# AutomationLabs-sh/AutomationLabsModelPredictiveControl.jl

Hardware: AMD Instinct MI355X
Metric: MPC steps/s (batch=4096, nx=12, nu=4, N=30) (higher is better)
Workload: dtype f64; 1 GPU; configs[1]: hover-linearised quadrotor nx=12 nu=4 N=30, 4096 instances per GPU, shared model, x0 amplitude classes 0.3/1.0/3.0 interleaved, cold start every step; batch_per_gpu=4096, global_batch=4096, seed=0x5eed0002, setup_ramp_steps=300, admm_max_iter=6, check_every=6, polish=1, warm_state_kept=False, parallelism=instances sharded over 1 GPU(s), 16-instance tile per workgroup

## Files before the change

automationlabsmodelpredictivecontrol.jl_amd/csrc/almpc_kernels.hip.h:

```cpp
#pragma once
#include <hip/hip_runtime.h>
#include <stdint.h>

#include <map>
#include <mutex>
#include <utility>
#include <type_traits>

namespace almpc {

inline hipError_t ensure_dyn_lds(const void* fn, size_t bytes) {
    if (bytes <= 64 * 1024) return hipSuccess;
    static std::mutex mu;
    static std::map<std::pair<int, const void*>, size_t> cur;
    int dev = 0;
    hipError_t e = hipGetDevice(&dev);
    if (e != hipSuccess) return e;
    std::lock_guard<std::mutex> lock(mu);
    size_t& c = cur[std::make_pair(dev, fn)];
    if (c >= bytes) return hipSuccess;
    e = hipFuncSetAttribute(fn, hipFuncAttributeMaxDynamicSharedMemorySize, (int)bytes);
    if (e == hipSuccess) c = bytes;
    return e;
}
// ... 587 lines not shown
    const double f = piv ? -invd : col * invd;
    const double keep = piv ? 0.0 : 1.0;
#pragma unroll
    for (int jj = 0; jj < 16; ++jj) r[jj] = __builtin_fma(-f, pj[jj], keep * r[jj]);
    if (own) r[JJ] = f;
}

template <int JJ>
__device__ __forceinline__ void gj16_pivot2(gj16_row& r, const double (&pj0)[16], const double (&pj1)[16], const double col0, const double col1,
                                            const double i11, const double t, const double s22, const bool own, const int k, const int lane) {
    static_assert((JJ & 1) == 0 && JJ + 1 < 16, "a pair starts at an even position");
    const double e11 = fast_rcp_d(s22);
    const double e01 = -t * e11;
    const double e00 = __builtin_fma(-t, e01, i11);
    const bool p0 = lane == k, p1 = lane == k + 1;
    double f0 = __builtin_fma(col0, e00, col1 * e01), f1 = __builtin_fma(col0, e01, col1 * e11);
    f0 = p0 ? -e00 : (p1 ? -e01 : f0);
    f1 = p0 ? -e01 : (p1 ? -e11 : f1);
    const double keep = (p0 || p1) ? 0.0 : 1.0;
#pragma unroll
    for (int jj = 0; jj < 16; ++jj) r[jj] = __builtin_fma(-f1, pj1[jj], __builtin_fma(-f0, pj0[jj], keep * r[jj]));
    if (own) { r[JJ] = f0; r[JJ + 1] = f1; }
}

template <int I, int N, class F>
__device__ __forceinline__ void gj_static_for(F&& f) {
    if constexpr (I < N) {
        if (!f(std::integral_constant<int, I>{})) return;
        gj_static_for<I + 1, N>(f);
    }
}

__device__ __forceinline__ void wave_lds_sync() {
    __builtin_amdgcn_fence(__ATOMIC_RELEASE, "workgroup");
    __builtin_amdgcn_wave_barrier();
    __builtin_amdgcn_fence(__ATOMIC_ACQUIRE, "workgroup");
}

template <int CTRL, int ROW_MASK>
__device__ __forceinline__ double dpp_d(double v) {
    int lo = __double2loint(v), hi = __double2hiint(v);
    lo = __builtin_amdgcn_update_dpp(lo, lo, CTRL, ROW_MASK, 0xF, false);
    hi = __builtin_amdgcn_update_dpp(hi, hi, CTRL, ROW_MASK, 0xF, false);
    return __hiloint2double(hi, lo);
}
#define ALMPC_WAVE_REDUCE(NAME, OP)                                                     \
    __device__ __forceinline__ double NAME(double v) {                                  \
        v = OP(v, dpp_d<0x121, 0xF>(v));                                 \
        v = OP(v, dpp_d<0x122, 0xF>(v));                                 \
        v = OP(v, dpp_d<0x124, 0xF>(v));                                 \
        v = OP(v, dpp_d<0x128, 0xF>(v));                                 \
        { const double o = dpp_d<0x142, 0xA>(v);           \
          const bool take = ((threadIdx.x >> 4) & 1) != 0; v = take ? OP(v, o) : v; }   \
        { const double o = dpp_d<0x143, 0xC>(v);           \
          const bool take = ((threadIdx.x >> 5) & 1) != 0; v = take ? OP(v, o) : v; }   \
        return readlane_d(v, 63);                                                       \
    }
__device__ __forceinline__ double op_add(double a, double b) { return a + b; }
__device__ __forceinline__ double op_min(double a, double b) { return fmin(a, b); }
__device__ __forceinline__ double op_max(double a, double b) { return fmax(a, b); }
ALMPC_WAVE_REDUCE(wave_sum, op_add)
ALMPC_WAVE_REDUCE(wave_min, op_min)
ALMPC_WAVE_REDUCE(wave_max, op_max)
#undef ALMPC_WAVE_REDUCE

__device__ __forceinline__ double half_sum(double v) {
    const unsigned lo = (unsigned)__double2loint(v), hi = (unsigned)__double2hiint(v);
    const auto a = __builtin_amdgcn_permlane32_swap(lo, lo, false, false);
    const auto b = __builtin_amdgcn_permlane32_swap(hi, hi, false, false);
    return __hiloint2double((int)b[0], (int)a[0]) + __hiloint2double((int)b[1], (int)a[1]);
}

__device__ __forceinline__ void lds_barrier() {
    __builtin_amdgcn_fence(__ATOMIC_RELEASE, "workgroup", "local");
    __builtin_amdgcn_s_barrier();
    __builtin_amdgcn_fence(__ATOMIC_ACQUIRE, "workgroup", "local");
}

template <class T>
__device__ __forceinline__ T* GL(T* q) {
    return (T*)(__attribute__((address_space(1))) T*)q;
}

__device__ __forceinline__ void wave_fence_lds() {
    __builtin_amdgcn_fence(__ATOMIC_RELEASE, "wavefront");
    __builtin_amdgcn_wave_barrier();
    __builtin_amdgcn_fence(__ATOMIC_ACQUIRE, "wavefront");
}

struct RowMultOut {
    double* mu = nullptr;
    const int* done = nullptr;
    const double* mer = nullptr;
};
__device__ __forceinline__ bool row_mult_live(const RowMultOut& r, int inst) {
    return r.mu != nullptr && !(r.done && r.done[inst] != 0) && !(r.mer && r.mer[4 * (size_t)inst + 2] != 0.0);
}

template <bool GLB>
struct PolishMode {
    static constexpr bool glb = GLB;
    static constexpr bool half = !GLB;
    static constexpr int WL = GLB ? 64 : 32;
    static constexpr int PMASK = WL - 1;
};

template <int CPL>
__device__ __forceinline__ void rollout_steps(double* Z, int n, int m, int N, int G, int lane, const double* A,
                                              const double* B) {
    const int C = n + m;
    const int i = lane / G, g = lane % G;
    double coef[CPL];
    int jc[CPL];
#pragma unroll
    for (int t = 0; t < CPL; ++t) {
        const int j = g * CPL + t;
        const bool ok = (i < n) && (j < C);
        const int ic = i < n ? i : 0;
        const double av = A[(size_t)(j < n ? j : 0) * n + ic], bv = B[(size_t)((j >= n && j < C) ? j - n : 0) * n + ic];
        coef[t] = ok ? (j < n ? av : bv) : 0.0;
        jc[t] = j < C ? j : C - 1;
    }
    for (int k = 0; k < N; ++k) {
        const double* zk = Z + (size_t)k * C;
        double zv[CPL];
#pragma unroll
        for (int t = 0; t < CPL; ++t) zv[t] = zk[jc[t]];
        double acc = 0.0;
#pragma unroll
        for (int t = 0; t < CPL; ++t) acc += coef[t] * zv[t];
        if (G == 4) {
            acc += dpp_d<0xB1, 0xF>(acc);
            acc += dpp_d<0x4E, 0xF>(acc);
        } else {
            for (int o = 1; o < G; o <<= 1) acc += __shfl_xor(acc, o);
        }
        if (g == 0 && i < n) Z[(size_t)(k + 1) * C + i] = acc;
        __builtin_amdgcn_fence(__ATOMIC_RELEASE, "wavefront");
        __builtin_amdgcn_wave_barrier();
        __builtin_amdgcn_fence(__ATOMIC_ACQUIRE, "wavefront");
    }
}

constexpr int ROLL_SMX = 24, ROLL_NX = 16;
template <int SMX, int NX>
__device__ __forceinline__ void roll_load(const double* M, int lane, double (&cu)[SMX], double (&cx)[NX]) {
#pragma unroll
    for (int c = 0; c < SMX; ++c) cu[c] = M[c * 64 + lane];
#pragma unroll
    for (int c = 0; c < NX; ++c) cx[c] = M[(ROLL_SMX + c) * 64 + lane];
}
template <int SMX, int NX>
__device__ __forceinline__ void roll_run(const double (&cu)[SMX], const double (&cx)[NX], int n, int m, int N, int s, int nb, int lane,
                                         const double* eub, double e0v, double x0r, const double* xref_lds, const double* xref_glb,
                                         double* gx, double* gex) {
    const int nx = n * (N + 1), sm = s * m;
    if (lane < n) {
        gex[lane] = e0v;
        if (gx) gx[lane] = x0r;
    }
    const bool mine = lane < s * n;
    auto upart = [&](int b, double (&acc)[4]) {
        const double* ub = eub + b * sm;
        double uv[SMX];
#pragma unroll
        for (int c = 0; c < SMX; ++c) uv[c] = ub[c];
#pragma unroll
        for (int t = 0; t < 4; ++t) acc[t] = 0.0;
#pragma unroll
        for (int c = 0; c < SMX; ++c) acc[c & 3] = __builtin_fma(cu[c], uv[c], acc[c & 3]);
    };
    double acc[4];
    upart(0, acc);
    double prev = e0v;
    int src0 = 0;
#pragma unroll 1
    for (int b = 0; b < nb; ++b) {
        const int t = (b * s + 1) * n + lane;
        const bool ok = mine && t < nx;
        const int tc = ok ? t : 0;
        double xr;
        if (xref_lds) xr = xref_lds[tc];
        else xr = xref_glb[tc];
#pragma unroll
        for (int c = 0; c < NX; ++c) {
            const int sl = src0 + c;
            acc[c & 3] = __builtin_fma(cx[c], readlane_d(prev, sl < 64 ? sl : 63), acc[c & 3]);
        }
        const double ev = (acc[0] + acc[1]) + (acc[2] + acc[3]);
        prev = ev;
        src0 = (s - 1) * n;
        upart(b + 1, acc);
        if (xref_lds) asm volatile("" : "+v"(xr));
        if (ok) {
            gex[t] = ev;
            if (gx) gx[t] = ev + xr;
        }
    }
}

constexpr int POLISH_WAVES = 4;
#ifndef ALMPC_EXP_POLISH_WAVES
#define ALMPC_EXP_POLISH_WAVES 8
#endif
constexpr int POLISH_WAVES_GLDS = ALMPC_EXP_POLISH_WAVES;
constexpr int POLISH_LDS_MIN_PER_WAVE = 128 + 64 + 64 + 32;
struct PolishShared {
    int off_d, off_umin, off_umax, off_uref, off_ab, off_xref, total;
};
__host__ __device__ inline PolishShared polish_shared_layout(int n, int m, int N, int nz, int nzs, int fused) {
    PolishShared L;
    L.off_d = 0;
    L.off_umin = nzs;
    L.off_umax = L.off_umin + m;
    L.off_uref = L.off_umax + m;
    L.off_ab = L.off_uref + nz;
    L.off_xref = L.off_ab + ((fused && fused != 3) ? n * (n + m) : 0);
    L.total = (L.off_xref + (fused ? (N + 1) * n : 0) + 1) & ~1;
    return L;
}
constexpr int POLISH_GLB_PER_INST = 64 * 64;
constexpr int POLISH_SG_SHARED_CAP = 48;
constexpr int HANDOFF_REC = POLISH_LDS_MIN_PER_WAVE;
static_assert((TILE - 8) * HANDOFF_REC <= POLISH_SG_SHARED_CAP * 64, "the records of ranks 8..15 must fit the second-tier slot");

typedef double d2 __attribute__((ext_vector_type(2)));

template <bool GLDS, bool GPRE, int KOFF, bool SGL = false, bool START = false>
__device__ __forceinline__ void polish_body(const PolishParams& p_arg, double* smem) {
    const PolishParams& p = p_arg;
    constexpr int CH = (GLDS || SGL) ? 8 : 16;
    constexpr int NWV = GLDS ? POLISH_WAVES_GLDS : (SGL ? 1 : POLISH_WAVES);
    const int wv = __builtin_amdgcn_readfirstlane(threadIdx.x >> 6), lane_k = threadIdx.x & 63;
    const int nz = p.nz, nzs = p.nzs;
    const double* Gp = p.G;
    const int gs = GLDS ? ((nz + 1) & ~1) : nzs;
    const PolishShared SL = polish_shared_layout(p.roll.n, p.m, p.roll.N, nz, nzs, p.fuse_rollout);
    double* shc = smem + (GLDS ? (size_t)nz * gs : 0);
    double* wave_lds = shc + SL.total + (size_t)wv * p.lds_per_wave;
    int* qcnt = nullptr;
    const bool uref_sh = p.uref_stride == 0, xref_sh = p.roll.xref_stride == 0;
    const bool per_inst = p.G_stride != 0;
    double* cd = shc + SL.off_d;
    double* cab = shc + SL.off_ab;
    if (per_inst) { cd = wave_lds + p.wave_const_off; cab = cd + nzs; }
    bool handed = false;
    if constexpr (GLDS && GPRE) handed = p.handoff != 0;
    if (!handed) {
        constexpr int TPB = 64 * NWV;
        const int n = p.roll.n, m = p.m, N = p.roll.N;
        if (!per_inst)
            for (int t = threadIdx.x; t < nzs; t += TPB) shc[SL.off_d + t] = p.dvec[t];
        for (int t = threadIdx.x; t < m; t += TPB) { shc[SL.off_umin + t] = p.umin[t]; shc[SL.off_umax + t] = p.umax[t]; }
        if (uref_sh)
            for (int t = threadIdx.x; t < nz; t += TPB) shc[SL.off_uref + t] = p.uref[t];
        if (p.fuse_rollout) {
            if (!per_inst && p.fuse_rollout != 3) {
                for (int t = threadIdx.x; t < n * n; t += TPB) shc[SL.off_ab + t] = p.roll.A[t];
                for (int t = threadIdx.x; t < n * m; t += TPB) shc[SL.off_ab + n * n + t] = p.roll.B[t];
            }
            if (xref_sh)
                for (int t = threadIdx.x; t < (N + 1) * n; t += TPB) shc[SL.off_xref + t] = p.roll.xref[t];
        }
    }
    ALMPC_STAMP(8192 + blockIdx.x * 8 + wv, 0);
    if constexpr (GLDS && !GPRE) {
        const int hs = gs / 2;
        const bool lane_in = lane_k < hs;
        const int lq = lane_in ? lane_k : 0;
        for (int r0_ = wv; r0_ < nz; r0_ += POLISH_WAVES_GLDS * 8) {
            d2 v[8];
#pragma unroll
            for (int u = 0; u < 8; ++u) {
                const int r = r0_ + u * POLISH_WAVES_GLDS;
                v[u] = *reinterpret_cast<const d2*>(p.G + (size_t)(r < nz ? r : 0) * nzs + 2 * lq);
            }
#pragma unroll
            for (int u = 0; u < 8; ++u) {
                const int r = r0_ + u * POLISH_WAVES_GLDS;
                if (r < nz && lane_in) *reinterpret_cast<d2*>(smem + (size_t)r * gs + 2 * lq) = v[u];
            }
        }
    }
    if constexpr (GLDS) {
        qcnt = reinterpret_cast<int*>(shc + SL.total + (size_t)POLISH_WAVES_GLDS * p.lds_per_wave);
        if (!handed && threadIdx.x == 0) { qcnt[0] = POLISH_WAVES_GLDS; qcnt[1] = -1; qcnt[2] = 0; }
        Gp = smem;
    }
    if (!handed) __syncthreads();
#ifdef ALMPC_EXP_LANE_GEOMETRY_PER_INSTANCE
    constexpr bool GEO_ONCE = false;
#else
    constexpr bool GEO_ONCE = CH == 8;
#endif
    [[maybe_unused]] int geo_m0 = 0;
    if constexpr (GEO_ONCE) geo_m0 = (2 * lane_k) % p.m;
  auto process = [&](const int inst, const double* rec, const int rank) {
    auto ka_ = __builtin_amdgcn_kernarg_segment_ptr();
    asm volatile("" : "+s"(ka_));
    const PolishParams& p = *(const PolishParams*)((const char*)ka_ + KOFF);
    int lane = lane_k;
    asm volatile("" : "+v"(lane));
    ALMPC_STAMP(inst, 8);
    if constexpr (!GLDS) {
        if (per_inst) {
            if constexpr (SGL) {
                double* gl = wave_lds + p.g_off;
                const char* src = reinterpret_cast<const char*>(GL(p.G) + (size_t)inst * p.G_stride) + lane * 16;
                if (lane < nzs / 2)
                    for (int r = 0; r < nz; ++r)
                        __builtin_amdgcn_global_load_lds((const __attribute__((address_space(1))) void*)(src + (size_t)r * nzs * 8),
                                                         (__attribute__((address_space(3))) void*)(gl + (size_t)r * nzs), 16, 0, 0);
                Gp = gl;
            } else
            Gp = GL(p.G) + (size_t)inst * p.G_stride;
            const int n_ = p.roll.n, m_ = p.m;
            for (int t = lane; t < nzs; t += 64) cd[t] = GL(p.dvec)[(size_t)inst * p.d_stride + t];
            if (p.fuse_rollout) {
                for (int t = lane; t < n_ * n_; t += 64) cab[t] = GL(p.roll.A)[(size_t)inst * p.A_stride + t];
                for (int t = lane; t < n_ * m_; t += 64) cab[n_ * n_ + t] = GL(p.roll.B)[(size_t)inst * p.B_stride + t];
            }
            if constexpr (SGL) __builtin_amdgcn_s_waitcnt(0);
            wave_fence_lds();
        }
    }
    bool from_rec = false;
    if constexpr (GLDS && GPRE) from_rec = rec != nullptr;
    int st_in;
    if (from_rec) st_in = __builtin_amdgcn_readfirstlane(reinterpret_cast<const int*>(rec + 256)[HANDOFF_STATUS]);
    else st_in = GL(p.status)[inst];
    const size_t base = (size_t)inst * nzs;
    const int r0 = 2 * lane, r1 = 2 * lane + 1;
    const bool in0 = r0 < nz, in1 = r1 < nz;
    const bool inrow = r0 < nzs;
    const int rc = inrow ? r0 : 0;
    const bool skip = (st_in == 2);
    int im0;
    if constexpr (GEO_ONCE) im0 = geo_m0; else im0 = r0 % p.m;
    const int im1 = (im0 + 1 == p.m) ? 0 : im0 + 1;

    double* rowbuf = wave_lds;
    double* pbufa = rowbuf + 128;
    double* pbufb = pbufa + 64;
    int* wrow_s = reinterpret_cast<int*>(pbufb + 64);
#ifdef ALMPC_EXP_ROW_NUMBERS
    auto woff = [&](int row) { return row; };
    auto wadr = [&](int e) { return e * gs; };
#else
    auto woff = [&](int row) { return row * gs; };
    auto wadr = [&](int e) { return e; };
#endif
    double* Sg;
    int cap2 = 64;
    bool own_slot = false;
    const bool sg_lds = SGL && p.sg_off >= 0;
    if (sg_lds) Sg = wave_lds + p.sg_off;
    else Sg = GL(p.sglobal) + (size_t)inst * POLISH_GLB_PER_INST;

    double lo0 = 0, hi0 = 0, lo1 = 0, hi1 = 0, v00, v01, w0 = 0, w1 = 0, y0, y1, z0, z1;
    double x0r = 0.0;
    if (p.fuse_rollout && lane < p.roll.n) x0r = GL(p.roll.x0)[(size_t)inst * p.roll.n + lane];
    {
        const d2 dv = *reinterpret_cast<const d2*>(cd + rc);
        d2 vv, yy, zz;
        if (from_rec) {
            const int o = (rc + handoff_rot(rank)) & 127;
            zz = *reinterpret_cast<const d2*>(rec + o);
            vv = *reinterpret_cast<const d2*>(rec + 128 + o);
            uint32_t wd = (uint32_t)reinterpret_cast<const int*>(rec + 256)[rc >> 4];
            asm volatile("" : "+v"(zz), "+v"(vv), "+v"(wd));
            const uint32_t b = (uint32_t)(rc & 15);
            yy[0] = (double)(int)((wd >> (16u + b)) & 1u) - (double)(int)((wd >> b) & 1u);
            yy[1] = (double)(int)((wd >> (17u + b)) & 1u) - (double)(int)((wd >> (b + 1u)) & 1u);
            if (rank >= POLISH_WAVES_GLDS) {
                __builtin_amdgcn_fence(__ATOMIC_RELEASE, "workgroup");
                if (lane == 0) atomicSub(qcnt + 2, 1);
// ... 508 lines not shown
                        pbufa[hpos] = Sr[tj];
                        pbufb[hpos] = (hpos < pv) ? -Sr[tj] : Sr[tj];
                    }
                    wave_fence_lds();
                    const double fcol = pbufa[hpos], piv = pbufa[pv];
                    double rowpv[16];
                    bcast16(pbufb, rowpv);
                    const double ip = fast_rcp_d(piv);
                    const bool isp = hpos == pv;
                    const double f = isp ? 0.0 : fcol * ip;
                    const double scale = isp ? ip : 1.0;
#pragma unroll
                    for (int t = 0; t < 16; ++t) Sr[t] = __builtin_fma(-f, rowpv[t], Sr[t]) * scale;
                    Sr[tj] = (hhf == hh) ? (isp ? ip : -f) : Sr[tj];
                }
            }
        }
        recompute(m);
        if (pass == 1 || k0 > 32) break;
        {
            const bool mine = lane < 32 && pos < k;
            const double viol = mine ? ((wsd > 0) ? -lam : lam) : -__builtin_inf();
            const double lmax = wave_max(mine ? fabs(lam) : 0.0);
            const bool bad = mine && viol > 1e-12 * fmax(1.0, lmax);
            const unsigned badm = (unsigned)__ballot(bad);
            const int nb = __popc(badm);
            if (nb < 2) break;
            const unsigned usedm = (k >= 32) ? 0xffffffffu : ((1u << k) - 1u);
            const unsigned keepm = usedm & ~badm;
            put_rows(0.0, 0.0);
            if (bad) rowbuf[wrow] = 1.0;
            wave_fence_lds();
            {
                const d2 mk = *reinterpret_cast<const d2*>(rowbuf + r0);
                if (mk[0] != 0.0) act0 = false;
                if (mk[1] != 0.0) act1 = false;
            }
            const bool keep = lane < 32 && ((keepm >> pos) & 1u) != 0u;
            const int np = __popc(keepm & ((1u << pos) - 1u));
            if (keep) { ibuf[np] = wrow; ibuf[64 + np] = wsd; pbufa[np] = wbnd; }
            wave_fence_lds();
            k = __popc(keepm);
            wrow = 0; wsd = 0; wbnd = 0.0; lam = 0.0;
            if (pos < k) { wrow = ibuf[pos]; wsd = ibuf[64 + pos]; wbnd = pbufa[pos]; }
            wave_fence_lds();
            it += nb;
        }
        }
        if (k0 > 32) {
            tier2_home(k0);
            to_global();
            for (int q = 32; q < k0; ++q)
                add_row(PolishMode<true>{}, __builtin_amdgcn_readlane(pend_row, q), readlane_d(pend_bnd, q),
                        __builtin_amdgcn_readlane(pend_sd, q));
            fresh = false;
            overflow = true;
        }
        }
    }
    ALMPC_STAMP(inst, 10);
    if (!give_up) {
        if (!overflow) {
            run(PolishMode<false>{});
            if (overflow) { tier2_home(33); to_global(); }
        }
        if (overflow) {
            overflow = false;
            run(PolishMode<true>{});
            if (overflow && own_slot) {
                slot_to_global();
                overflow = false;
                run(PolishMode<true>{});
            }
            give_up = overflow;
        }
    }
    if constexpr (GLDS) {
        if (own_slot) {
            if (lane == 0) atomicExch(qcnt + 1, -1);
            own_slot = false;
        }
    }

    ALMPC_STAMP(inst, 11);
    ALMPC_ACC_FLUSH(inst);
    d2 wout;
    if (p.unsolved && lane == 0 && ((give_up || fin != 0) ? st_in : 0) != 0) {
        __hip_atomic_fetch_add(p.unsolved, 1, __ATOMIC_RELAXED, __HIP_MEMORY_SCOPE_SYSTEM);
        if (p.redo_gate) *GL(p.redo_gate) = p.step_serial;
    }
    if (give_up) {
        wout[0] = skip ? z0 : fmin(fmax(z0, lo0), hi0);
        wout[1] = skip ? z1 : fmin(fmax(z1, lo1), hi1);
    } else {
        wout[0] = act0 ? bnd0 : fmin(fmax(w0, lo0), hi0);
        wout[1] = act1 ? bnd1 : fmin(fmax(w1, lo1), hi1);
        if (lane == 0) {
            GL(p.piters)[inst] = it;
            GL(p.status)[inst] = (fin == 0) ? 0 : st_in;
        }
    }
    if (p.dflag && lane == 0 && GL(p.dflag)[inst] != 0) GL(p.status)[inst] = 2;
    if (!p.fuse_rollout) {
        if (inrow) *reinterpret_cast<d2*>(GL(p.w) + base + r0) = wout;
        return;
    }
    {
        const RolloutParams& rp = p.roll;
        const int n = rp.n, m = rp.m, N = rp.N, C = n + m;
        double* Z = wave_lds;
        const d2 dvp = *reinterpret_cast<const d2*>(cd + rc);
        double ur0 = 0.0, ur1 = 0.0;
        if (uref_sh) {
            ur0 = shc[SL.off_uref + (in0 ? r0 : 0)];
            ur1 = shc[SL.off_uref + (in1 ? r1 : 0)];
            asm volatile("" : "+v"(ur0), "+v"(ur1));
        } else {
            const double* ug = GL(rp.uref) + (size_t)inst * rp.uref_stride;
            ur0 = ug[in0 ? r0 : 0];
            ur1 = ug[in1 ? r1 : 0];
        }
        if (p.fuse_rollout == 3) {
            const bool exact = p.roll_s * m <= 20 && n <= 12;
            double cu[ROLL_SMX], cx[ROLL_NX];
            if (exact) {
                double cu2[20], cx2[12];
                roll_load<20, 12>(GL(p.rollM), lane, cu2, cx2);
#pragma unroll
                for (int c = 0; c < ROLL_SMX; ++c) cu[c] = c < 20 ? cu2[c] : 0.0;
#pragma unroll
                for (int c = 0; c < ROLL_NX; ++c) cx[c] = c < 12 ? cx2[c] : 0.0;
            } else {
                roll_load<ROLL_SMX, ROLL_NX>(GL(p.rollM), lane, cu, cx);
            }
            const int m0 = im0, m1 = im1;
            double e0 = 0.0, e1 = 0.0;
            if (in0) {
                const double uu = fmin(fmax(wout[0] * dvp[0] + ur0, shc[SL.off_umin + m0]), shc[SL.off_umax + m0]);
                e0 = uu - ur0;
                GL(rp.u)[(size_t)inst * nz + r0] = uu;
                GL(rp.eu)[(size_t)inst * nz + r0] = e0;
            }
            if (in1) {
                const double uu = fmin(fmax(wout[1] * dvp[1] + ur1, shc[SL.off_umin + m1]), shc[SL.off_umax + m1]);
                e1 = uu - ur1;
                GL(rp.u)[(size_t)inst * nz + r1] = uu;
                GL(rp.eu)[(size_t)inst * nz + r1] = e1;
            }
            double* eub = wave_lds;
            {
                d2 ev; ev[0] = e0; ev[1] = e1;
                *reinterpret_cast<d2*>(eub + 2 * lane) = ev;
                d2 zz; zz[0] = 0.0; zz[1] = 0.0;
                *reinterpret_cast<d2*>(eub + 128 + 2 * lane) = zz;
            }
            double e0v = 0.0;
            const double* xg = nullptr;
            if (lane < n) {
                double xr0;
                if (xref_sh) { xr0 = shc[SL.off_xref + lane]; asm volatile("" : "+v"(xr0)); }
                else xr0 = GL(rp.xref)[(size_t)inst * rp.xref_stride + lane];
                e0v = x0r - xr0;
            }
            if (!xref_sh) xg = GL(rp.xref) + (size_t)inst * rp.xref_stride;
            wave_fence_lds();
            ALMPC_STAMP(inst, 12);
            const size_t xo3 = (size_t)inst * n * (N + 1);
            double* gx = GL(rp.x) + xo3;
            double* gex = GL(rp.ex) + xo3;
            const double* xl = xref_sh ? (shc + SL.off_xref) : nullptr;
            if (exact) {
                double cu2[20], cx2[12];
#pragma unroll
                for (int c = 0; c < 20; ++c) cu2[c] = cu[c];
#pragma unroll
                for (int c = 0; c < 12; ++c) cx2[c] = cx[c];
                roll_run<20, 12>(cu2, cx2, n, m, N, p.roll_s, p.roll_nb, lane, eub, e0v, x0r, xl, xg, gx, gex);
            } else {
                roll_run<ROLL_SMX, ROLL_NX>(cu, cx, n, m, N, p.roll_s, p.roll_nb, lane, eub, e0v, x0r, xl, xg, gx, gex);
            }
            ALMPC_STAMP(inst, 13);
            ALMPC_STAMP(inst, 14);
            return;
        }
        const int m0 = im0, m1 = im1, k0s = r0 / m, k1s = (m0 + 1 == m) ? k0s + 1 : k0s;
        if (in0) {
            const double uu = fmin(fmax(wout[0] * dvp[0] + ur0, shc[SL.off_umin + m0]), shc[SL.off_umax + m0]);
            GL(rp.u)[(size_t)inst * nz + r0] = uu;
            GL(rp.eu)[(size_t)inst * nz + r0] = uu - ur0;
            Z[(size_t)k0s * C + n + m0] = uu - ur0;
        }
        if (in1) {
            const double uu = fmin(fmax(wout[1] * dvp[1] + ur1, shc[SL.off_umin + m1]), shc[SL.off_umax + m1]);
            GL(rp.u)[(size_t)inst * nz + r1] = uu;
            GL(rp.eu)[(size_t)inst * nz + r1] = uu - ur1;
            Z[(size_t)k1s * C + n + m1] = uu - ur1;
        }
        if (p.fuse_rollout == 2) return;
        if (lane < n) {
            double xr0;
            if (xref_sh) { xr0 = shc[SL.off_xref + lane]; asm volatile("" : "+v"(xr0)); }
            else xr0 = GL(rp.xref)[(size_t)inst * rp.xref_stride + lane];
            Z[lane] = x0r - xr0;
        }
        wave_fence_lds();
        ALMPC_STAMP(inst, 12);
        switch (p.roll_cpl) {
            case 1: rollout_steps<1>(Z, n, m, N, p.roll_g, lane, cab, cab + n * n); break;
            case 2: rollout_steps<2>(Z, n, m, N, p.roll_g, lane, cab, cab + n * n); break;
            case 4: rollout_steps<4>(Z, n, m, N, p.roll_g, lane, cab, cab + n * n); break;
            default: rollout_steps<8>(Z, n, m, N, p.roll_g, lane, cab, cab + n * n); break;
        }
        ALMPC_STAMP(inst, 13);
        const int nx = n * (N + 1);
        const size_t xo = (size_t)inst * nx;
        const float inv_n = 1.0f / (float)n;
        for (int t0 = 0; t0 < nx; t0 += 4 * 64) {
            double ev[4], xr[4];
            int tt[4];
#pragma unroll
            for (int u = 0; u < 4; ++u) {
                const int t = t0 + 64 * u + lane;
                tt[u] = t < nx ? t : nx - 1;
                const int kq = (int)(((float)tt[u] + 0.5f) * inv_n);
                ev[u] = Z[(size_t)tt[u] + (size_t)kq * m];
            }
            if (xref_sh) {
#pragma unroll
                for (int u = 0; u < 4; ++u) xr[u] = shc[SL.off_xref + tt[u]];
                asm volatile("" : "+v"(xr[0]), "+v"(xr[1]), "+v"(xr[2]), "+v"(xr[3]));
            } else {
                const double* xg = GL(rp.xref) + (size_t)inst * rp.xref_stride;
#pragma unroll
                for (int u = 0; u < 4; ++u) xr[u] = xg[tt[u]];
            }
#pragma unroll
            for (int u = 0; u < 4; ++u) {
                const int t = t0 + 64 * u + lane;
                if (t < nx) {
                    GL(rp.ex)[xo + t] = ev[u];
                    GL(rp.x)[xo + t] = (t < n) ? x0r : ev[u] + xr[u];
                }
            }
        }
        ALMPC_STAMP(inst, 14);
    }
  };

    if constexpr (GLDS) {
        ALMPC_STAMP(8192 + blockIdx.x * 8 + wv, 1);
        [[maybe_unused]] int nproc = 0;
        for (int i = wv;;) {
            const int tile = (i >> 4) * (int)gridDim.x + (int)blockIdx.x;
            if (tile >= p.ntiles) break;
            int inst;
            const double* rec = nullptr;
            if (handed) {
                if (i >= p.batch - (int)blockIdx.x * TILE) break;
                rec = i < POLISH_WAVES_GLDS ? wave_lds : shc + p.sg_shared_off + (size_t)(i - POLISH_WAVES_GLDS) * HANDOFF_REC;
                inst = __builtin_amdgcn_readfirstlane(reinterpret_cast<const int*>(rec + 256)[HANDOFF_INST]);
            } else {
                inst = p.perm[tile * 16 + (i & 15)];
            }
            if (inst >= 0) {
                process(inst, rec, i);
                ++nproc;
// ... 185 lines not shown
```

automationlabsmodelpredictivecontrol.jl_amd/csrc/almpc_polish_gen.hip.h:

```cpp
#pragma once
#include "almpc_kernels.hip.h"

namespace almpc {

struct PolishGenParams {
    int nz, mc, R, Rs, m, n, N, batch, nzs;
    const double* Ghat;
    const double* gnorm;
    long Ghat_stride = 0, gnorm_stride = 0, d_stride = 0, A_stride = 0, B_stride = 0;
    int ltv = 0;
    const double* ltvA = nullptr;
    const double* ltvB = nullptr;
    const double* ltvC = nullptr;
    const double* eq_off = nullptr;
    long eq_stride = 0;
    const double* rollM = nullptr;
    int roll_s = 0, roll_nb = 0;
    int eq_proj = 0, eq0 = 0, ne = 0;
    const double* GhatE = nullptr;
    const double* WinvE = nullptr;
    const int* row_traj;
    const int* row_eq;
    const int* row_xidx;
    const int* row_state;
// ... 742 lines not shown
    if (lane == 0) {
        p.piters[inst] = it;
        const int st_out = (st_in == 2) ? 2 : ((fin == 0) ? 0 : (fin == 3 ? 3 : 1));
        p.status[inst] = st_out;
        const bool requeue = !QUEUE && overflow && fin != 3;
        if (requeue) p.ovf[2 + atomicAdd(p.ovf, 1)] = inst;
        if (p.unsolved && st_out == 1 && !requeue) {
            __hip_atomic_fetch_add(p.unsolved, 1, __ATOMIC_RELAXED, __HIP_MEMORY_SCOPE_SYSTEM);
            if (p.redo_gate) *p.redo_gate = p.step_serial;
        }
    }
    if (p.redo_ws) {
        const int st_out = (st_in == 2) ? 2 : ((fin == 0) ? 0 : (fin == 3 ? 3 : 1));
        const bool requeue = !QUEUE && overflow && fin != 3;
        int32_t* rw = p.redo_ws + (size_t)inst * 64;
        if (st_out == 1 && !requeue && k > 0) {
            const int pos = WL == 32 ? (lane & 31) : lane;
            if (lane < WL && pos < k && pos < 63) {
                const int xi = p.row_xidx[wrow];
                const int t = wrow < p.nz ? (wrow / p.m) * p.redo_sp + p.redo_nt + wrow % p.m : (xi / p.n) * p.redo_sp + xi % p.n;
                rw[1 + pos] = (t << 2) | (wsd == 0 ? 2 : (wsd > 0 ? 1 : 0));
            }
            if (lane == 0) rw[0] = k < 63 ? k : 63;
        } else if (lane == 0) rw[0] = 0;
    }
    if (!QUEUE && overflow && fin != 3) {
        if (lane < 32) p.ovf_ws[(size_t)inst * 32 + lane] = guess_overflow ? -1 : (wrow | ((wsd + 1) << 12));
        if (p.ovf_sinv && !guess_overflow) {
            double* sv_ = p.ovf_sinv + (size_t)inst * (32 * 32 + 32);
#pragma unroll 4
            for (int t = 0; t < 32; t += 2) sv_[(t + (lane >> 5)) * 32 + (lane & 31)] = Sl[(t + (lane >> 5)) * WL + (lane & 31)];
            if (lane < 32) sv_[32 * 32 + lane] = wbnd;
        }
    }
    wave_fence_lds();
    if (p.rows.mu && fin == 0 && st_in != 2 && row_mult_live(p.rows, inst)) {
#pragma unroll
        for (int q = 0; q < NP; ++q) {
            d2 v; v[0] = 0.0; v[1] = 0.0;
            *reinterpret_cast<d2*>(rowbuf + 2 * lane + 128 * q) = v;
        }
        wave_fence_lds();
        if (lowhalf && pos < k && wrow >= nz) rowbuf[wrow] = lam;
        wave_fence_lds();
        double* mo = p.rows.mu + (size_t)inst * N * n;
        for (int t = lane; t < N * n; t += 64) {
            const int r = p.rows_map[t];
            mo[t] = r >= 0 ? rowbuf[nz + r] : 0.0;
        }
        wave_fence_lds();
    }
    {
        const int r0 = 2 * lane, r1 = 2 * lane + 1;
        const int rc = (r0 < nzs) ? r0 : 0;
        const d2 dvp = *reinterpret_cast<const d2*>(dvi + rc);
        if (r0 < nz) {
            const double ur = rp.uref[(size_t)inst * rp.uref_stride + r0];
            const double uu = fmin(fmax(wout[0] * dvp[0] + ur, rp.umin[r0 % m]), rp.umax[r0 % m]);
            rp.u[(size_t)inst * nz + r0] = uu;
            rp.eu[(size_t)inst * nz + r0] = uu - ur;
            Z[(size_t)(r0 / m) * C + n + r0 % m] = uu - ur;
        }
        if (r1 < nz) {
            const double ur = rp.uref[(size_t)inst * rp.uref_stride + r1];
            const double uu = fmin(fmax(wout[1] * dvp[1] + ur, rp.umin[r1 % m]), rp.umax[r1 % m]);
            rp.u[(size_t)inst * nz + r1] = uu;
            rp.eu[(size_t)inst * nz + r1] = uu - ur;
            Z[(size_t)(r1 / m) * C + n + r1 % m] = uu - ur;
        }
        if (blocked) {
            {
                d2 ev;
                ev[0] = (r0 < nz) ? Z[(size_t)(r0 / m) * C + n + r0 % m] : 0.0;
                ev[1] = (r1 < nz) ? Z[(size_t)(r1 / m) * C + n + r1 % m] : 0.0;
                wave_fence_lds();
                *reinterpret_cast<d2*>(EUB + 2 * lane) = ev;
                d2 zz; zz[0] = 0.0; zz[1] = 0.0;
                *reinterpret_cast<d2*>(EUB + 128 + 2 * lane) = zz;
            }
            double e0v = 0.0, x0r = 0.0;
            if (lane < n) { x0r = rp.x0[(size_t)inst * n + lane]; e0v = x0r - rp.xref[(size_t)inst * rp.xref_stride + lane]; }
            double cu[ROLL_SMX], cx[ROLL_NX];
            roll_load<ROLL_SMX, ROLL_NX>(p.rollM, lane, cu, cx);
            wave_fence_lds();
            PGEN_STAMP(13);
            const size_t xo = (size_t)inst * n * (N + 1);
            roll_run<ROLL_SMX, ROLL_NX>(cu, cx, n, m, N, p.roll_s, p.roll_nb, lane, EUB, e0v, x0r, nullptr,
                                        rp.xref + (size_t)inst * rp.xref_stride, rp.x + xo, rp.ex + xo);
            PGEN_STAMP(14);
        } else if (!p.ltv) {
        for (int i = lane; i < n; i += 64) Z[i] = rp.x0[(size_t)inst * n + i] - rp.xref[(size_t)inst * rp.xref_stride + i];
        wave_fence_lds();
        PGEN_STAMP(13);
        roll(Z);
        PGEN_STAMP(14);
        const int nx = n * (N + 1);
        const size_t xo = (size_t)inst * nx;
        for (int t0 = 0; t0 < nx; t0 += 256) {
            double xr4[4];
#pragma unroll
            for (int j = 0; j < 4; ++j) {
                const int t = t0 + 64 * j + lane, tc = t < nx ? t : 0;
                xr4[j] = (tc < n) ? rp.x0[(size_t)inst * n + tc] : rp.xref[(size_t)inst * rp.xref_stride + tc];
            }
#pragma unroll
            for (int j = 0; j < 4; ++j) {
                const int t = t0 + 64 * j + lane;
                if (t < nx) {
                    const double ev = Z[(size_t)(t / n) * C + t % n];
                    rp.ex[xo + t] = ev;
                    rp.x[xo + t] = (t < n) ? xr4[j] : ev + xr4[j];
                }
            }
        }
        }
    }
    PGEN_STAMP(6);
    if (QUEUE) wave_fence_lds();
  } while (QUEUE);
}

struct GhatInstParams {
    int n, m, N, nz, nzs, mc, R, Rs;
    const double* A; const double* B;
    long A_stride, B_stride;
    long A_kstride, B_kstride;
    const double* G; long G_stride;
    const double* dvec; long d_stride;
    const int* rowmap;
    double* Ghat; long Ghat_stride;
    double* gnorm; long gnorm_stride;
};
constexpr int GHAT_THREADS = 256;

template <int NX>
__global__ __launch_bounds__(GHAT_THREADS) void k_ghat_inst(GhatInstParams p) {
    extern __shared__ __attribute__((aligned(16))) double smem[];
    const int inst = blockIdx.x, tid = threadIdx.x;
    const int n = p.n, m = p.m, N = p.N, nz = p.nz, nzs = p.nzs, mc = p.mc, R = p.R, Rs = p.Rs;
    double* AB = smem;
    const double* G = p.G + (size_t)inst * p.G_stride;
    const double* dv = p.dvec + (size_t)inst * p.d_stride;
    double* Gh = p.Ghat + (size_t)inst * p.Ghat_stride;
    double* gn = p.gnorm + (size_t)inst * p.gnorm_stride;
    for (int t = tid; t < nz * nz; t += GHAT_THREADS) Gh[(size_t)(t / nz) * Rs + t % nz] = G[(size_t)(t / nz) * nzs + t % nz];
    for (int pass = 0; pass < 2; ++pass) {
        const int ncol = pass == 0 ? nz : mc;
        for (int c0 = 0; c0 < ncol; c0 += GHAT_THREADS) {
            const int c = c0 + tid;
            const bool on = c < ncol;
            const int cc = on ? c : 0;
            double x[NX];
#pragma unroll
            for (int i = 0; i < NX; ++i) x[i] = 0.0;
            for (int t = 0; t < N; ++t) {
                if (t == 0 || p.A_kstride != 0) {
                    __syncthreads();
                    const double* At = p.A + (size_t)inst * p.A_stride + (size_t)t * p.A_kstride;
                    const double* Bt = p.B + (size_t)inst * p.B_stride + (size_t)t * p.B_kstride;
                    for (int e = tid; e < n * n; e += GHAT_THREADS) AB[e] = At[e];
                    for (int e = tid; e < n * m; e += GHAT_THREADS) AB[n * n + e] = Bt[e];
                    __syncthreads();
                }
                double xn[NX];
#pragma unroll
                for (int i = 0; i < NX; ++i) xn[i] = 0.0;
#pragma unroll
                for (int j = 0; j < NX; ++j)
                    if (j < n) {
                        const double xj = x[j];
#pragma unroll
// ... 126 lines not shown
```

Baseline: 18700 batch-steps/s (one step = 4096 instance QP solves).

## Restructure fused polish rollout tail to overlap loads and prefetch xref

Moves the fuse_rollout==3 tail ahead of the status writes. It issues the rollout matrix loads early, hoists the kernel arguments into scalar registers once, and places a waitcnt before the tail so those loads overlap with the u/eu stores and status writes. roll_run now prefetches the next block's xref value one iteration ahead. It uses explicit global and LDS address-space pointers, with template tags replacing the runtime LDS/global branch. The exact-size register arrays are loaded directly instead of through copies into padded arrays. The risk is higher register pressure and subtle ordering issues around the waitcnt and the asm barriers.

```diff
diff --git a/automationlabsmodelpredictivecontrol.jl_amd/csrc/almpc_kernels.hip.h b/automationlabsmodelpredictivecontrol.jl_amd/csrc/almpc_kernels.hip.h
--- a/automationlabsmodelpredictivecontrol.jl_amd/csrc/almpc_kernels.hip.h
+++ b/automationlabsmodelpredictivecontrol.jl_amd/csrc/almpc_kernels.hip.h
@@ -693,6 +693,11 @@
     return (T*)(__attribute__((address_space(1))) T*)q;
 }
 
+template <class T>
+__device__ __forceinline__ __attribute__((address_space(1))) T* G1(T* q) {
+    return (__attribute__((address_space(1))) T*)q;
+}
+
 __device__ __forceinline__ void wave_fence_lds() {
     __builtin_amdgcn_fence(__ATOMIC_RELEASE, "wavefront");
     __builtin_amdgcn_wave_barrier();
@@ -757,20 +762,30 @@
 template <int SMX, int NX>
 __device__ __forceinline__ void roll_load(const double* M, int lane, double (&cu)[SMX], double (&cx)[NX]) {
 #pragma unroll
-    for (int c = 0; c < SMX; ++c) cu[c] = M[c * 64 + lane];
-#pragma unroll
-    for (int c = 0; c < NX; ++c) cx[c] = M[(ROLL_SMX + c) * 64 + lane];
-}
-template <int SMX, int NX>
+    for (int c = 0; c < SMX; ++c) cu[c] = G1(M)[c * 64 + lane];
+#pragma unroll
+    for (int c = 0; c < NX; ++c) cx[c] = G1(M)[(ROLL_SMX + c) * 64 + lane];
+}
+template <int NX>
+__device__ __forceinline__ void roll_arrived(double (&cx)[NX]) {
+#pragma unroll
+    for (int c = 0; c < NX; ++c) asm volatile("" : "+v"(cx[c]));
+}
+struct RollRefLds { const double* p; static constexpr bool lds = true; };
+struct RollRefGlb { const double* p; static constexpr bool lds = false; };
+template <int SMX, int NX, class XREF>
 __device__ __forceinline__ void roll_run(const double (&cu)[SMX], const double (&cx)[NX], int n, int m, int N, int s, int nb, int lane,
-                                         const double* eub, double e0v, double x0r, const double* xref_lds, const double* xref_glb,
-                                         double* gx, double* gex) {
-    const int nx = n * (N + 1), sm = s * m;
+                                         const double* eub, double e0v, double x0r, XREF xref, double* gx, double* gex) {
+    const int nx = n * (N + 1), sm = s * m, sn = s * n;
     if (lane < n) {
-        gex[lane] = e0v;
-        if (gx) gx[lane] = x0r;
-    }
-    const bool mine = lane < s * n;
+        G1(gex)[lane] = e0v;
+        G1(gx)[lane] = x0r;
+    }
+    const bool mine = lane < sn;
+    auto xref_at = [&](int i) -> double {
+        if constexpr (XREF::lds) return ((const __attribute__((address_space(3))) double*)xref.p)[i];
+        else return G1(xref.p)[i];
+    };
     auto upart = [&](int b, double (&acc)[4]) {
         const double* ub = eub + b * sm;
         double uv[SMX];
@@ -783,16 +798,13 @@
     };
     double acc[4];
     upart(0, acc);
+    int t = n + lane;
+    bool ok = mine && t < nx;
+    double xr = xref_at(ok ? t : 0);
     double prev = e0v;
     int src0 = 0;
 #pragma unroll 1
     for (int b = 0; b < nb; ++b) {
-        const int t = (b * s + 1) * n + lane;
-        const bool ok = mine && t < nx;
-        const int tc = ok ? t : 0;
-        double xr;
-        if (xref_lds) xr = xref_lds[tc];
-        else xr = xref_glb[tc];
 #pragma unroll
         for (int c = 0; c < NX; ++c) {
             const int sl = src0 + c;
@@ -802,11 +814,14 @@
         prev = ev;
         src0 = (s - 1) * n;
         upart(b + 1, acc);
-        if (xref_lds) asm volatile("" : "+v"(xr));
+        const int tn = t + sn;
+        const bool okn = mine && tn < nx;
+        const double xrn = xref_at(okn ? tn : 0);
         if (ok) {
-            gex[t] = ev;
-            if (gx) gx[t] = ev + xr;
-        }
+            G1(gex)[t] = ev;
+            G1(gx)[t] = ev + xr;
+        }
+        t = tn; ok = okn; xr = xrn;
     }
 }
 
@@ -903,6 +918,11 @@
     constexpr bool GEO_ONCE = false;
 #else
     constexpr bool GEO_ONCE = CH == 8;
+#endif
+#ifdef ALMPC_EXP_TAIL_ARGS_AT_USE
+    constexpr bool TAIL_ARGS_ONCE = false;
+#else
+    constexpr bool TAIL_ARGS_ONCE = CH == 8;
 #endif
     [[maybe_unused]] int geo_m0 = 0;
     if constexpr (GEO_ONCE) geo_m0 = (2 * lane_k) % p.m;
@@ -1577,6 +1597,7 @@
         }
     }
 
+    if constexpr (TAIL_ARGS_ONCE) __builtin_amdgcn_s_waitcnt(0x0F70);
     ALMPC_STAMP(inst, 11);
     ALMPC_ACC_FLUSH(inst);
     d2 wout;
@@ -1590,12 +1611,105 @@
     } else {
         wout[0] = act0 ? bnd0 : fmin(fmax(w0, lo0), hi0);
         wout[1] = act1 ? bnd1 : fmin(fmax(w1, lo1), hi1);
-        if (lane == 0) {
-            GL(p.piters)[inst] = it;
-            GL(p.status)[inst] = (fin == 0) ? 0 : st_in;
-        }
-    }
-    if (p.dflag && lane == 0 && GL(p.dflag)[inst] != 0) GL(p.status)[inst] = 2;
+    }
+    auto put_status = [&](int32_t* stp, int32_t* pip, const int* dfp) {
+        if (!give_up && lane == 0) {
+            G1(pip)[inst] = it;
+            G1(stp)[inst] = (fin == 0) ? 0 : st_in;
+        }
+        if (dfp && lane == 0 && G1(dfp)[inst] != 0) G1(stp)[inst] = 2;
+    };
+    if (p.fuse_rollout == 3) {
+        int a_fn = p.roll.n, a_fm = p.roll.m, a_fN = p.roll.N, a_rs = p.roll_s, a_rnb = p.roll_nb;
+        const double* a_rollM = p.rollM;
+        const double* a_xref = p.roll.xref;
+        const double* a_uref = p.roll.uref;
+        long a_xrs = p.roll.xref_stride, a_urs = p.roll.uref_stride;
+        double* a_x = p.roll.x;
+        double* a_ex = p.roll.ex;
+        double* a_u = p.roll.u;
+        double* a_eu = p.roll.eu;
+        int32_t* a_status = p.status;
+        int32_t* a_piters = p.piters;
+        const int* a_dflag = p.dflag;
+        if constexpr (TAIL_ARGS_ONCE) {
+            asm volatile("" : "+s"(a_fn), "+s"(a_fm), "+s"(a_fN), "+s"(a_rs), "+s"(a_rnb), "+s"(a_rollM), "+s"(a_xref), "+s"(a_uref),
+                         "+s"(a_xrs), "+s"(a_urs));
+        }
+        const int n = a_fn, m = a_fm, N = a_fN, rs = a_rs, rnb = a_rnb;
+        const int inst_s = __builtin_amdgcn_readfirstlane(inst);
+        const size_t uo = (size_t)inst_s * nz, xo3 = (size_t)inst_s * n * (N + 1);
+        auto tail = [&](auto& cu, auto& cx, auto run) __attribute__((always_inline)) {
+            roll_load(a_rollM, lane, cu, cx);
+            const d2 dvp = *reinterpret_cast<const d2*>(cd + rc);
+            double ur0, ur1;
+            if (uref_sh) {
+                ur0 = shc[SL.off_uref + (in0 ? r0 : 0)];
+                ur1 = shc[SL.off_uref + (in1 ? r1 : 0)];
+                asm volatile("" : "+v"(ur0), "+v"(ur1));
+            } else {
+                const auto* ug = G1(a_uref) + (size_t)inst_s * a_urs;
+                ur0 = ug[in0 ? r0 : 0];
+                ur1 = ug[in1 ? r1 : 0];
+                asm volatile("" : "+v"(ur0), "+v"(ur1));
+            }
+            const double uu0 = fmin(fmax(wout[0] * dvp[0] + ur0, shc[SL.off_umin + im0]), shc[SL.off_umax + im0]);
+            const double uu1 = fmin(fmax(wout[1] * dvp[1] + ur1, shc[SL.off_umin + im1]), shc[SL.off_umax + im1]);
+            const double e0 = in0 ? uu0 - ur0 : 0.0, e1 = in1 ? uu1 - ur1 : 0.0;
+            double* eub = wave_lds;
+            {
+                d2 ev; ev[0] = e0; ev[1] = e1;
+                *reinterpret_cast<d2*>(eub + 2 * lane) = ev;
+                d2 zz; zz[0] = 0.0; zz[1] = 0.0;
+                *reinterpret_cast<d2*>(eub + 128 + 2 * lane) = zz;
+            }
+            const int lc = lane < n ? lane : 0;
+            const double* xl = shc + SL.off_xref;
+            const double* xg = a_xref + (size_t)inst_s * a_xrs;
+            double xr0;
+            if (xref_sh) {
+                xr0 = xl[lc];
+                asm volatile("" : "+v"(xr0));
+            } else {
+                xr0 = G1(xg)[lc];
+                asm volatile("" : "+v"(xr0));
+            }
+            const double e0v = lane < n ? x0r - xr0 : 0.0;
+            if constexpr (TAIL_ARGS_ONCE) roll_arrived(cx);
+            if (in0) {
+                G1(a_u)[uo + r0] = uu0;
+                G1(a_eu)[uo + r0] = e0;
+            }
+            if (in1) {
+                G1(a_u)[uo + r1] = uu1;
+                G1(a_eu)[uo + r1] = e1;
+            }
+            put_status(a_status, a_piters, a_dflag);
+            if constexpr (!TAIL_ARGS_ONCE) roll_arrived(cx);
+            wave_fence_lds();
+            ALMPC_STAMP(inst, 12);
+            double* gx = a_x + xo3;
+            double* gex = a_ex + xo3;
+            if (xref_sh) run(eub, e0v, RollRefLds{xl}, gx, gex);
+            else run(eub, e0v, RollRefGlb{xg}, gx, gex);
+            ALMPC_STAMP(inst, 13);
+            ALMPC_STAMP(inst, 14);
+        };
+        const bool exact = p.roll_s * m <= 20 && n <= 12;
+        if (exact) {
+            double cu2[20], cx2[12];
+            tail(cu2, cx2, [&](const double* eub, double e0v, auto xr, double* gx, double* gex) __attribute__((always_inline)) {
+                roll_run<20, 12>(cu2, cx2, n, m, N, rs, rnb, lane, eub, e0v, x0r, xr, gx, gex);
+            });
+        } else {
+            double cu[ROLL_SMX], cx[ROLL_NX];
+            tail(cu, cx, [&](const double* eub, double e0v, auto xr, double* gx, double* gex) __attribute__((always_inline)) {
+                roll_run<ROLL_SMX, ROLL_NX>(cu, cx, n, m, N, rs, rnb, lane, eub, e0v, x0r, xr, gx, gex);
+            });
+        }
+        return;
+    }
+    put_status(p.status, p.piters, p.dflag);
     if (!p.fuse_rollout) {
         if (inrow) *reinterpret_cast<d2*>(GL(p.w) + base + r0) = wout;
         return;
@@ -1614,69 +1728,6 @@
             const double* ug = GL(rp.uref) + (size_t)inst * rp.uref_stride;
             ur0 = ug[in0 ? r0 : 0];
             ur1 = ug[in1 ? r1 : 0];
-        }
-        if (p.fuse_rollout == 3) {
-            const bool exact = p.roll_s * m <= 20 && n <= 12;
-            double cu[ROLL_SMX], cx[ROLL_NX];
-            if (exact) {
-                double cu2[20], cx2[12];
-                roll_load<20, 12>(GL(p.rollM), lane, cu2, cx2);
-#pragma unroll
-                for (int c = 0; c < ROLL_SMX; ++c) cu[c] = c < 20 ? cu2[c] : 0.0;
-#pragma unroll
-                for (int c = 0; c < ROLL_NX; ++c) cx[c] = c < 12 ? cx2[c] : 0.0;
-            } else {
-                roll_load<ROLL_SMX, ROLL_NX>(GL(p.rollM), lane, cu, cx);
-            }
-            const int m0 = im0, m1 = im1;
-            double e0 = 0.0, e1 = 0.0;
-            if (in0) {
-                const double uu = fmin(fmax(wout[0] * dvp[0] + ur0, shc[SL.off_umin + m0]), shc[SL.off_umax + m0]);
-                e0 = uu - ur0;
-                GL(rp.u)[(size_t)inst * nz + r0] = uu;
-                GL(rp.eu)[(size_t)inst * nz + r0] = e0;
-            }
-            if (in1) {
-                const double uu = fmin(fmax(wout[1] * dvp[1] + ur1, shc[SL.off_umin + m1]), shc[SL.off_umax + m1]);
-                e1 = uu - ur1;
-                GL(rp.u)[(size_t)inst * nz + r1] = uu;
-                GL(rp.eu)[(size_t)inst * nz + r1] = e1;
-            }
-            double* eub = wave_lds;
-            {
-                d2 ev; ev[0] = e0; ev[1] = e1;
-                *reinterpret_cast<d2*>(eub + 2 * lane) = ev;
-                d2 zz; zz[0] = 0.0; zz[1] = 0.0;
-                *reinterpret_cast<d2*>(eub + 128 + 2 * lane) = zz;
-            }
-            double e0v = 0.0;
-            const double* xg = nullptr;
-            if (lane < n) {
-                double xr0;
-                if (xref_sh) { xr0 = shc[SL.off_xref + lane]; asm volatile("" : "+v"(xr0)); }
-                else xr0 = GL(rp.xref)[(size_t)inst * rp.xref_stride + lane];
-                e0v = x0r - xr0;
-            }
-            if (!xref_sh) xg = GL(rp.xref) + (size_t)inst * rp.xref_stride;
-            wave_fence_lds();
-            ALMPC_STAMP(inst, 12);
-            const size_t xo3 = (size_t)inst * n * (N + 1);
-            double* gx = GL(rp.x) + xo3;
-            double* gex = GL(rp.ex) + xo3;
-            const double* xl = xref_sh ? (shc + SL.off_xref) : nullptr;
-            if (exact) {
-                double cu2[20], cx2[12];
-#pragma unroll
-                for (int c = 0; c < 20; ++c) cu2[c] = cu[c];
-#pragma unroll
-                for (int c = 0; c < 12; ++c) cx2[c] = cx[c];
-                roll_run<20, 12>(cu2, cx2, n, m, N, p.roll_s, p.roll_nb, lane, eub, e0v, x0r, xl, xg, gx, gex);
-            } else {
-                roll_run<ROLL_SMX, ROLL_NX>(cu, cx, n, m, N, p.roll_s, p.roll_nb, lane, eub, e0v, x0r, xl, xg, gx, gex);
-            }
-            ALMPC_STAMP(inst, 13);
-            ALMPC_STAMP(inst, 14);
-            return;
         }
         const int m0 = im0, m1 = im1, k0s = r0 / m, k1s = (m0 + 1 == m) ? k0s + 1 : k0s;
         if (in0) {
diff --git a/automationlabsmodelpredictivecontrol.jl_amd/csrc/almpc_polish_gen.hip.h b/automationlabsmodelpredictivecontrol.jl_amd/csrc/almpc_polish_gen.hip.h
--- a/automationlabsmodelpredictivecontrol.jl_amd/csrc/almpc_polish_gen.hip.h
+++ b/automationlabsmodelpredictivecontrol.jl_amd/csrc/almpc_polish_gen.hip.h
@@ -848,11 +848,12 @@
             if (lane < n) { x0r = rp.x0[(size_t)inst * n + lane]; e0v = x0r - rp.xref[(size_t)inst * rp.xref_stride + lane]; }
             double cu[ROLL_SMX], cx[ROLL_NX];
             roll_load<ROLL_SMX, ROLL_NX>(p.rollM, lane, cu, cx);
+            roll_arrived(cx);
             wave_fence_lds();
             PGEN_STAMP(13);
             const size_t xo = (size_t)inst * n * (N + 1);
-            roll_run<ROLL_SMX, ROLL_NX>(cu, cx, n, m, N, p.roll_s, p.roll_nb, lane, EUB, e0v, x0r, nullptr,
-                                        rp.xref + (size_t)inst * rp.xref_stride, rp.x + xo, rp.ex + xo);
+            roll_run<ROLL_SMX, ROLL_NX>(cu, cx, n, m, N, p.roll_s, p.roll_nb, lane, EUB, e0v, x0r,
+                                        RollRefGlb{rp.xref + (size_t)inst * rp.xref_stride}, rp.x + xo, rp.ex + xo);
             PGEN_STAMP(14);
         } else if (!p.ltv) {
         for (int i = lane; i < n; i += 64) Z[i] = rp.x0[(size_t)inst * n + i] - rp.xref[(size_t)inst * rp.xref_stride + i];
```

Measured after the change: 18770 batch-steps/s (one step = 4096 instance QP solves) (median of 6 runs). No clear change (+0.4%).
